# jibanCat/gp_dla_detection

Hardware: AMD Instinct MI355X
Metric: sample log-likelihoods/sec (n~1500,k=20) (higher is better)
Workload: dtype f64; 1 GPU; BASELINE configs[1]: synthetic spectra, fused Voigt + low-rank log-evidence sweep, HBM-resident; spectra_per_gpu=1000, pixels=1500, k=20, dla_samples=10000, num_lines=3, parallelism=spectra sharded over 1 GPU(s), RCCL all-gather of the 15-column posterior table

## Files before the change

gp_dla_detection_amd/_lib.py:

```python
from __future__ import annotations

import ctypes as C
import os
import subprocess

_HERE = os.path.dirname(os.path.abspath(__file__))
CSRC = os.path.join(_HERE, "csrc")
DEFAULT_LIB_PATH = os.path.join(CSRC, "libgpdla.so")


def lib_path() -> str:
    return os.environ.get("GPDLA_LIB_PATH") or DEFAULT_LIB_PATH

HIPCC_FLAGS = ["--offload-arch=gfx950", "-O3", "-ffp-contract=off", "-fPIC", "-shared",
               "-std=c++17", "-no-hip-rt", "-Wno-inline-asm"]

LEGACY_LIB_PATH = os.path.join(CSRC, "libgpdla_legacy.so")

_dp = C.POINTER(C.c_double)
_i64p = C.POINTER(C.c_int64)
_i32p = C.POINTER(C.c_int32)
_u8p = C.POINTER(C.c_uint8)
_u32p = C.POINTER(C.c_uint32)

# ... 146 lines not shown
    ("gpdla_batch_samples_device_ptr", C.c_int, [C.c_void_p, C.POINTER(C.c_void_p), _i64p, _i64p]),
    ("gpdla_context_last_sweep_ms", C.c_double, [C.c_void_p]),
    ("gpdla_context_set_timing", C.c_int, [C.c_void_p, C.c_int]),
    ("gpdla_process_batch_multi", C.c_int, [C.POINTER(Model), C.POINTER(Samples), C.POINTER(Spectra),
                                            _u32p, C.POINTER(Config), C.POINTER(ResultsMulti), C.c_int]),
    ("gpdla_batch_process_multi", C.c_int, [C.c_void_p, C.c_void_p, _u32p]),
    ("gpdla_batch_download_multi", C.c_int, [C.c_void_p, C.c_void_p, C.POINTER(ResultsMulti)]),
    ("gpdla_batch_summary_multi_device_ptr", C.c_int, [C.c_void_p, C.POINTER(C.c_void_p), _i64p, _i32p]),
    ("gpdla_batch_samples_multi_device_ptr", C.c_int, [C.c_void_p, C.POINTER(C.c_void_p),
                                                       C.POINTER(C.c_void_p), C.POINTER(C.c_void_p)]),
    ("gpdla_training_create", C.c_int, [C.c_int, C.c_int64, C.c_int64, _dp, _dp, _dp,
                                        C.POINTER(C.c_void_p)]),
    ("gpdla_training_objective", C.c_int, [C.c_void_p, _dp, C.c_int, _dp, _dp]),
    ("gpdla_training_set_lyseries", C.c_int, [C.c_void_p, C.c_int, _dp, _dp]),
    ("gpdla_training_destroy", None, [C.c_void_p]),
    ("gpdla_training_create_from_spectra", C.c_int, [C.c_int, C.POINTER(Spectra), C.POINTER(LearnConfig),
                                                     C.POINTER(C.c_void_p)]),
    ("gpdla_training_column_stats", C.c_int, [C.c_void_p, _dp, _dp, _i64p]),
    ("gpdla_training_pca_covariance", C.c_int, [C.c_void_p, C.c_int, _dp, _dp, _i64p]),
    ("gpdla_training_download", C.c_int, [C.c_void_p, _dp, _dp, _dp]),
    ("gpdla_stats_bin_posteriors", C.c_int, [C.c_int64, C.c_int64, _dp, C.c_int64, _dp, _dp, _dp, _dp, _dp, _dp, _dp,
                                             C.c_int, C.POINTER(BinRequest), C.POINTER(BinOutput), C.c_int]),
    ("gpdla_stats_poisson_binomial_cf", C.c_int, [C.c_int64, _i64p, _dp, _dp, _dp, C.c_int]),
    ("gpdla_model_spectra_validate", C.c_int, [C.POINTER(ModelSpectraRequest), C.c_int64, C.c_int64, C.c_int]),
    ("gpdla_batch_unmasked_counts", C.c_int, [C.c_void_p, C.c_void_p, _i64p]),
    ("gpdla_batch_model_spectra", C.c_int, [C.c_void_p, C.c_void_p, C.POINTER(ModelSpectraRequest),
                                            C.POINTER(ModelSpectra)]),
    ("gpdla_debug_profiles_ms", C.c_int, [C.c_void_p, C.c_void_p, _dp]),
    ("gpdla_model_mean", C.c_int, [C.POINTER(Model), C.c_int64, _dp, _i64p, _dp, _dp, C.c_int, C.c_int, C.c_int,
                                   C.c_double, C.c_double, _dp, C.c_int]),
    ("gpdla_mock_validate", C.c_int, [C.POINTER(MockRequest), C.c_int64]),
    ("gpdla_batch_draw_mocks", C.c_int, [C.c_void_p, C.c_void_p, C.POINTER(MockRequest), C.POINTER(MockSpectra)]),
    ("gpdla_debug_near_poly", C.c_int, [C.c_int, C.c_double, _dp, _dp]),
    ("gpdla_debug_prepared_rows", C.c_int, [C.c_void_p, C.c_void_p, C.c_int, C.c_int64, _dp, C.c_int64, _i64p]),
    ("gpdla_debug_philox4x32_10", None, [_u32p, _u32p, _u32p]),
    ("gpdla_debug_throw", C.c_int, [C.c_int]),
]

_lib = None


def host_sources() -> list:
    import re
    unit = os.path.join(CSRC, "gpdla.hip")
    with open(unit) as f:
        names = re.findall(r'^#include "(host_\w+\.hpp)"', f.read(), flags=re.M)
    return [unit] + [os.path.join(CSRC, n) for n in names]


def _build(out: str, extra_flags, force: bool, verbose: bool) -> str:
    import glob
    srcs = (host_sources() + glob.glob(os.path.join(CSRC, "*.hip")) + glob.glob(os.path.join(CSRC, "*.hpp"))
            + glob.glob(os.path.join(_HERE, "..", "include", "*.h")))
    if not force and os.path.exists(out):
        if all(os.path.getmtime(out) >= os.path.getmtime(s) for s in srcs):
            return out
    cmd = ["hipcc", *HIPCC_FLAGS, *extra_flags, os.path.join(CSRC, "gpdla.hip"), "-o", out]
    res = subprocess.run(cmd, capture_output=True, text=True)
    if verbose or res.returncode:
        print(res.stdout, res.stderr)
    if res.returncode:
        raise RuntimeError(f"hipcc failed building {os.path.basename(out)}:\n" + res.stderr)
    return out


def build(force: bool = False, verbose: bool = False) -> str:
# ... 49 lines not shown
```

gp_dla_detection_amd/csrc/host_common.hpp:

```cpp
#pragma once

namespace {

thread_local std::string t_error = "";

int fail(int code, const char *fmt, ...) {
  char buf[512];
  va_list ap;
  va_start(ap, fmt);
  vsnprintf(buf, sizeof(buf), fmt, ap);
  va_end(ap);
  t_error = buf;
  return code;
}

#define GPDLA_NO_THROW                                                                                    \
  catch (const std::bad_alloc &) { return fail(GPDLA_ERR_HOST, "out of host memory"); }                   \
  catch (const std::exception &e) { return fail(GPDLA_ERR_HOST, "unexpected C++ exception: %s", e.what()); } \
  catch (...) { return fail(GPDLA_ERR_HOST, "unexpected C++ exception"); }

#define HIP_TRY(expr)                                                                      \
  do {                                                                                     \
    hipError_t e_ = (expr);                                                                \
    if (e_ != hipSuccess)                                                                  \
// ... 37 lines not shown
  HIP_TRY(hipMalloc(reinterpret_cast<void **>(&d_near), g_near_host.size() * sizeof(double)));
  HIP_TRY(hipMemcpy(d_near, g_near_host.data(), g_near_host.size() * sizeof(double), hipMemcpyHostToDevice));
  LineTable t;
  t.near_poly = d_near;
#define GP_WL(i, wl, f, G, lead, gam) wl,
#define GP_LEAD(i, wl, f, G, lead, gam) lead,
#define GP_GAM(i, wl, f, G, lead, gam) gam,
#define GP_OSC(i, wl, f, G, lead, gam) f,
  const double wl[] = {GPDLA_LYMAN_SERIES(GP_WL)};
  const double lead[] = {GPDLA_LYMAN_SERIES(GP_LEAD)};
  const double gam[] = {GPDLA_LYMAN_SERIES(GP_GAM)};
  const double osc[] = {GPDLA_LYMAN_SERIES(GP_OSC)};
  const double taps[] = GPDLA_INSTRUMENT_PROFILE;
  const double sigma = GPDLA_GAUSS_SIGMA_CGS;
  for (int i = 0; i < kMaxLines; ++i) {
    t.wavelength_cm[i] = wl[i];
    t.leading[i] = lead[i];
    t.osc[i] = osc[i];
    t.y[i] = gam[i] / std::sqrt(2.0) / sigma;
    t.y2[i] = t.y[i] * t.y[i];
    t.cwing[i] = lead[i] * t.y[i];
    t.t2[i] = kE2 - 2.0 * t.y2[i];
    t.wing[i] = {GPDLA_SPEED_OF_LIGHT_CGS / wl[i] / 1e8 / (std::sqrt(2.0) * sigma), t.y2[i], t.cwing[i], 0.0};
  }
  for (int i = 0; i < 7; ++i) t.taps[i] = taps[i];
  t.c = GPDLA_SPEED_OF_LIGHT_CGS;
  t.inv_sqrt2_sigma = 1.0 / (std::sqrt(2.0) * sigma);
  t.inv_sqrt2pi_sigma = 1.0 / (std::sqrt(2.0 * 3.14159265358979323846) * sigma);
  HIP_TRY(hipMemcpyToSymbol(HIP_SYMBOL(g_lines), &t, sizeof(t)));
  if (device_id < 64) g_table_loaded[device_id] = true;
  return GPDLA_OK;
}

template <typename T>
int dev_alloc(T **p, size_t count) {
  *p = nullptr;
  if (count == 0) count = 1;
  HIP_TRY(hipMalloc(reinterpret_cast<void **>(p), count * sizeof(T)));
  return GPDLA_OK;
}

template <typename T>
int upload(T **p, const T *host, size_t count, hipStream_t st) {
  int rc = dev_alloc(p, count);
  if (rc) return rc;
  if (count) HIP_TRY(hipMemcpyAsync(*p, host, count * sizeof(T), hipMemcpyHostToDevice, st));
  return GPDLA_OK;
}

void dev_free(void *p) {
  if (p) (void)hipFree(p);
}

struct StreamDrain {
  hipStream_t stream;
  ~StreamDrain() { (void)hipStreamSynchronize(stream); }
};

template <typename T>
int reserve(T **p, size_t *cap, size_t count) {
  if (count == 0) count = 1;
  if (*p && *cap >= count) return GPDLA_OK;
  dev_free(*p);
  *p = nullptr;
  *cap = 0;
  int rc = dev_alloc(p, count);
// ... 60 lines not shown
```

gp_dla_detection_amd/csrc/host_sweep.hpp:

```cpp
#pragma once

namespace {

template <typename Args>
int launch_sweep_kernel(gpdla_context *c, void (*kernel)(Args), int threads, size_t lds, int samples_per_block,
                        int64_t num_quasars, Args args) {
  HIP_TRY(hipFuncSetAttribute(reinterpret_cast<const void *>(kernel), hipFuncAttributeMaxDynamicSharedMemorySize, (int)lds));
  args.blocks_per_quasar = (int32_t)((args.S + 1 + samples_per_block - 1) / samples_per_block);
  const int64_t nblocks = 8 * ((num_quasars + 7) / 8) * (int64_t)args.blocks_per_quasar;
  if (nblocks > 2147483647LL) return fail(GPDLA_ERR_UNSUPPORTED, "batch too large for one launch");
  hipLaunchKernelGGL(kernel, dim3((unsigned)nblocks), dim3(threads), lds, c->stream, args);
  HIP_TRY(hipGetLastError());
  return GPDLA_OK;
}

template <class F>
int dispatch_nd(int mode, F &&f) {
  switch (mode == 0 ? 1 : mode) {
    case 1: return f(std::integral_constant<int, 1>{});
    case 2: return f(std::integral_constant<int, 2>{});
    case 3: return f(std::integral_constant<int, 3>{});
    case 4: return f(std::integral_constant<int, 4>{});
    default: return fail(GPDLA_ERR_UNSUPPORTED, "max_dlas = %d > 4", mode);
  }
// ... 313 lines not shown
  if (k > 256) return fail(GPDLA_ERR_UNSUPPORTED, "k = %d too large", k);
  int rc = select_device(device_id);
  if (rc) return rc;
  double *buf = nullptr;
  const size_t nn = (size_t)n, ws = (size_t)k * (k + 1) / 2 + k + 2;
  const size_t n_in = 3 * nn + nn * k, total = n_in + ws + 2;
  if ((rc = dev_alloc(&buf, total))) return rc;
  std::vector<double> host(n_in);
  std::memcpy(host.data(), y, nn * sizeof(double));
  std::memcpy(host.data() + nn, mu, nn * sizeof(double));
  std::memcpy(host.data() + 2 * nn, d, nn * sizeof(double));
  std::memcpy(host.data() + 3 * nn, M, nn * k * sizeof(double));
  double *dy = buf, *dmu = dy + nn, *dd = dmu + nn, *dM = dd + nn, *dws = dM + nn * k, *dlp = dws + ws;
  int *d_status = reinterpret_cast<int *>(dlp + 1);
  hipError_t e = hipMemcpy(buf, host.data(), n_in * sizeof(double), hipMemcpyHostToDevice);
  double back[2] = {NAN, 0.0};
  if (e == hipSuccess) {
    hipLaunchKernelGGL(k_lowrank_single, dim3(1), dim3(256), 0, 0, dy, dmu, dM, dd, n, k, dws, dlp, d_status);
    e = hipGetLastError();
  }
  if (e == hipSuccess) e = hipMemcpy(back, dlp, 2 * sizeof(double), hipMemcpyDeviceToHost);
  dev_free(buf);
  if (e != hipSuccess) return fail(GPDLA_ERR_HIP, "gpdla_log_mvnpdf_low_rank: %s", hipGetErrorString(e));
  int status;
  std::memcpy(&status, &back[1], sizeof(int));
  *log_p = back[0];
  if (status) {
    *log_p = NAN;
    return fail(GPDLA_ERR_NOT_POSITIVE_DEFINITE, "B = I + M' D^-1 M is not positive definite");
  }
  return GPDLA_OK;
} GPDLA_NO_THROW

}

extern "C" int gpdla_debug_prepared_rows(gpdla_context *c, gpdla_batch *b, int multi, int64_t quasar,
                                         double *rows_out, int64_t capacity_rows, int64_t *num_rows_out) {
  if (!c || !b || b->ctx != c || !rows_out || !num_rows_out)
    return fail(GPDLA_ERR_INVALID_ARGUMENT, "null/mismatched argument");
  if (quasar < 0 || quasar >= b->nq) return fail(GPDLA_ERR_INVALID_ARGUMENT, "quasar %lld outside the batch", (long long)quasar);
  HIP_TRY(hipSetDevice(c->device_id));
  int rc = plan_records(c, b, b->k <= 20 ? kSlimRec : record_doubles(b->ntiles, 0), true);
  if (rc) return rc;
  if ((rc = launch_prepare(c, b, multi != 0))) return rc;
  QuasarMeta m;
  HIP_TRY(hipMemcpyAsync(&m, b->d_meta + quasar, sizeof(m), hipMemcpyDeviceToHost, c->stream));
  HIP_TRY(hipStreamSynchronize(c->stream));
  const int64_t n = std::min<int64_t>(m.n_u, capacity_rows);
  static_assert(sizeof(PixelRow) == 4 * sizeof(double), "rows_out is [n][4] doubles");
  if (n > 0) {
    HIP_TRY(hipMemcpyAsync(rows_out, b->d_pix + m.pix_off, (size_t)n * sizeof(PixelRow), hipMemcpyDeviceToHost, c->stream));
    HIP_TRY(hipStreamSynchronize(c->stream));
  }
  *num_rows_out = n;
  return GPDLA_OK;
}

#ifdef GPDLA_STAMP
extern "C" int gpdla_debug_stamps(unsigned long long *out) {
  unsigned long long zero[8] = {0, 0, 0, 0, 0, 0, 0, 0};
  if (hipDeviceSynchronize() != hipSuccess) return -1;
  if (hipMemcpyFromSymbol(out, HIP_SYMBOL(gpdla::g_stamps), sizeof(zero)) != hipSuccess) return -1;
  if (hipMemcpyToSymbol(HIP_SYMBOL(gpdla::g_stamps), zero, sizeof(zero)) != hipSuccess) return -1;
  return 0;
}
#endif
// ... 1 lines not shown
```

gp_dla_detection_amd/csrc/sweep_kernels.hpp:

```cpp
#pragma once
#include <hip/hip_runtime.h>
#include <stdint.h>

#include <type_traits>
#include <utility>

#include "faddeeva.hpp"
#include "near_tables.hpp"

namespace gpdla {

typedef double d4 __attribute__((ext_vector_type(4)));

typedef float f4 __attribute__((ext_vector_type(4)));

template <typename T> struct Mat;
template <> struct Mat<double> {
  using acc_t = d4;
  static __device__ __forceinline__ acc_t mfma(double a, double b, acc_t c) {
    return __builtin_amdgcn_mfma_f64_16x16x4f64(a, b, c, 0, 0, 0);
  }
  static __device__ __forceinline__ int sample_of(int jj, int r) { return jj + 4 * r; }
  static __device__ __forceinline__ int jj_of(int sample) { return sample & 3; }
  static __device__ __forceinline__ int reg_of(int sample) { return sample >> 2; }
};
template <> struct Mat<float> {
  using acc_t = f4;
  static __device__ __forceinline__ acc_t mfma(float a, float b, acc_t c) {
    return __builtin_amdgcn_mfma_f32_16x16x4f32(a, b, c, 0, 0, 0);
  }
  static __device__ __forceinline__ int sample_of(int jj, int r) { return 4 * jj + r; }
  static __device__ __forceinline__ int jj_of(int sample) { return sample >> 2; }
  static __device__ __forceinline__ int reg_of(int sample) { return sample & 3; }
};

constexpr int kMaxLines = 31;
constexpr int kSamplesPerWave = 16;
constexpr double kLog2Pi = 1.83787706640934534;

struct LineTable {
  double wavelength_cm[kMaxLines];
// ... 376 lines not shown
  int32_t blocks_per_quasar;
  int32_t k, tiles_w, ntiles, num_lines;
  double *sample_ll;
  double *ll_no_dla;
};

__device__ __forceinline__ double fast_rcp(double a) {
  const double r = __builtin_amdgcn_rcp(a);
  const double e = fma(-a, r, 1.0);
  return fma(r, e, r);
}

__device__ __forceinline__ double exp_nonpos(double x) {
  x = fmax(x, -800.0);
  const double n = rint(x * 1.4426950408889634);
  double r = fma(-n, 0.6931471803691238, x);
  r = fma(-n, 1.9082149292705877e-10, r);
  double p = 2.08767569878681e-09;
  p = fma(p, r, 2.505210838544172e-08);
  p = fma(p, r, 2.755731922398589e-07);
  p = fma(p, r, 2.755731922398589e-06);
  p = fma(p, r, 2.48015873015873e-05);
  p = fma(p, r, 0.0001984126984126984);
  p = fma(p, r, 0.001388888888888889);
  p = fma(p, r, 0.008333333333333333);
  p = fma(p, r, 0.041666666666666664);
  p = fma(p, r, 0.16666666666666666);
  p = fma(p, r, 0.5);
  p = fma(p, r, 1.0);
  p = fma(p, r, 1.0);
  return ldexp(p, (int)n);
}

constexpr double kE1 = 0x1.8000000000236p+0, kE2 = 0x1.dffffffd2a557p+1, kE3 = 0x1.a4000aa13fb7fp+3,
                 kE4 = 0x1.d86dfb645a1cbp+5, kE5 = 0x1.4be1ccccccccdp+8;

__device__ __forceinline__ double wing_core(double x2, double y2) {
  const double rho = fast_rcp(x2 + y2);
  double t = fma(kE5, rho, kE4);
  t = fma(t, rho, kE3);
  t = fma(t, rho, kE2);
  t = fma(t, rho, kE1);
  t = fma(t, rho, 1.0);
  t = fma(-2.0 * y2 * rho, rho, t);
  return rho * t;
}

__device__ __forceinline__ void glds16(const double *gsrc, double *lds_wave_base) {
  const uint32_t lds = __builtin_amdgcn_readfirstlane(
      (uint32_t)(uintptr_t)(__attribute__((address_space(3))) void *)lds_wave_base);
  asm volatile("s_mov_b32 m0, %1\n\ts_nop 0\n\tglobal_load_lds_dwordx4 %0, off"
               :
               : "v"(gsrc), "s"(lds)
               : "memory", "m0");
}
__device__ __forceinline__ void glds_wait() {
  __builtin_amdgcn_s_waitcnt(0x0F70);
  asm volatile("" ::: "memory");
}

constexpr int kRecordPoolPad = 8;
__device__ __forceinline__ void glds_quad(const double *gsrc, uint32_t lds, int count) {
  if (count >= 4)
    asm volatile("s_mov_b32 m0, %1\n\ts_nop 0\n\tglobal_load_lds_dwordx4 %0, off\n\t"
                 "global_load_lds_dwordx4 %0, off offset:1024\n\tglobal_load_lds_dwordx4 %0, off offset:2048\n\t"
                 "global_load_lds_dwordx4 %0, off offset:3072"
                 :
                 : "v"(gsrc), "s"(lds)
// ... 465 lines not shown
__device__ __forceinline__ uint32_t hi_word(double v) { return (uint32_t)__double2hiint(v); }

__device__ __forceinline__ double wing_sum3(double lamP, double msa, double msb, double msc, double cs,
                                            bool *near) {
  const double xa = fma(lamP, msa, -cs), xb = fma(lamP, msb, -cs), xc = fma(lamP, msc, -cs);
  const double sa = fma(xa, xa, g_lines.y2[0]), sb = fma(xb, xb, g_lines.y2[1]), sc = fma(xc, xc, g_lines.y2[2]);
  static_assert(__builtin_bit_cast(unsigned long long, 900.0) == 0x408C200000000000ull, "bits of 900.0");
  *near = min(min(hi_word(sa), hi_word(sb)), hi_word(sc)) < 0x408C2000u;
  const double pab = sa * sb, pbc = sb * sc, pac = sa * sc;
  const double rinv = fast_rcp(pab * sc);
  const double ra = rinv * pbc, rb = rinv * pac, rc = rinv * pab;
  double ta = ra * kE5 + kE4, tb = rb * kE5 + kE4, tc = rc * kE5 + kE4;
  ta = fma(ta, ra, kE3); tb = fma(tb, rb, kE3); tc = fma(tc, rc, kE3);
  ta = fma(ta, ra, g_lines.t2[0]); tb = fma(tb, rb, g_lines.t2[1]); tc = fma(tc, rc, g_lines.t2[2]);
  ta = fma(ta, ra, kE1); tb = fma(tb, rb, kE1); tc = fma(tc, rc, kE1);
  ta = fma(ta, ra, 1.0); tb = fma(tb, rb, 1.0); tc = fma(tc, rc, 1.0);
  return fma(g_lines.cwing[2], rc * tc, fma(g_lines.cwing[1], rb * tb, g_lines.cwing[0] * (ra * ta)));
}

__device__ __forceinline__ double wing_sum3_rcp4(double lamP, double msa, double msb, double msc, double cs,
                                                 bool *near, double d, double *inv_d) {
  const double xa = fma(lamP, msa, -cs), xb = fma(lamP, msb, -cs), xc = fma(lamP, msc, -cs);
  const double sa = fma(xa, xa, g_lines.y2[0]), sb = fma(xb, xb, g_lines.y2[1]), sc = fma(xc, xc, g_lines.y2[2]);
  *near = min(min(hi_word(sa), hi_word(sb)), hi_word(sc)) < 0x408C2000u;
  const double pab = sa * sb, pabc = pab * sc;
  const double rinv = fast_rcp(pabc * d);
  *inv_d = rinv * pabc;
  const double r3 = rinv * d;
  const double rc = r3 * pab, r2 = r3 * sc;
  const double ra = r2 * sb, rb = r2 * sa;
  double ta = ra * kE5 + kE4, tb = rb * kE5 + kE4, tc = rc * kE5 + kE4;
  ta = fma(ta, ra, kE3); tb = fma(tb, rb, kE3); tc = fma(tc, rc, kE3);
  ta = fma(ta, ra, g_lines.t2[0]); tb = fma(tb, rb, g_lines.t2[1]); tc = fma(tc, rc, g_lines.t2[2]);
  ta = fma(ta, ra, kE1); tb = fma(tb, rb, kE1); tc = fma(tc, rc, kE1);
  ta = fma(ta, ra, 1.0); tb = fma(tb, rb, 1.0); tc = fma(tc, rc, 1.0);
  return fma(g_lines.cwing[2], rc * tc, fma(g_lines.cwing[1], rb * tb, g_lines.cwing[0] * (ra * ta)));
}

constexpr int kRing2 = 33;
constexpr int kExpTab = 64;

struct ExpState {
  double r, tabv;
  int ni;
};
__device__ __forceinline__ ExpState exp_table_begin(double x, const double *tab) {
  ExpState e;
  const double nf = rint(x * 92.33248261689366);
  asm("v_cvt_i32_f64 %0, %1" : "=v"(e.ni) : "v"(nf));
  e.tabv = tab[e.ni & (kExpTab - 1)];
  e.r = fma(-nf, 0.010830424667801708, x);
  e.r = fma(-nf, 2.8447437476627285e-11, e.r);
  return e;
}
__device__ __forceinline__ double exp_table_end(const ExpState &e) {
  double p, c4 = 0.041666666666666664, c3 = 0.16666666666666666;
  asm("v_fma_f64 %0, %1, %2, %3" : "=v"(p) : "s"(0.008333333333333333), "v"(e.r), "v"(c4));
  asm("v_fma_f64 %0, %1, %2, %3" : "=v"(p) : "v"(p), "v"(e.r), "v"(c3));
  p = fma(p, e.r, 0.5);
  p = fma(p, e.r, 1.0);
  p = fma(p, e.r, 1.0);
  return ldexp(e.tabv * p, e.ni >> 6);
}
constexpr double kExpScale = 92.33248261689366;
__device__ __forceinline__ ExpState exp_table_begin_scaled(double t, const double *tab) {
  ExpState e;
// ... 591 lines not shown
```

gp_dla_detection_amd/csrc/sweep_slim_kernel.hpp:

```cpp
#pragma once
#include <type_traits>

#include "sweep_kernels.hpp"

namespace gpdla {

constexpr int kSlimExtras = 12;
constexpr int kSlimRec = 4 * kSlimExtras + 64;
constexpr int kSlimCH = 8;
constexpr int kSlimTilesW = 13;
constexpr int kSlimStepTiles = kSlimTilesW * 64;
constexpr int kSlimRingD = kSweepWaves * kSamplesPerWave * kRing2;
constexpr int kSlimTileBuf = kSlimCH * kSlimStepTiles;
constexpr int kSlimRawBuf = kSlimCH * kSlimRec;
constexpr int kSlimLand = 4 * 32 + 4 * 4;
constexpr int kSlimBlock = kSlimTileBuf + kSlimRawBuf;
constexpr int kSlimLdsDoubles = kSlimRingD + 2 * kSlimBlock + kSweepWaves * kSlimLand;
static_assert((kSlimBlock * 8) % 512 == 0, "both parities reachable with ds_read2st64 offsets");
static_assert(kSlimLdsDoubles * 8 == 160 * 1024, "the slim sweep uses the whole LDS of a CU");
static_assert((kSlimCH * kSlimRec) % 128 == 0, "a raw chunk is a whole number of KiB");

__host__ __device__ constexpr int slim_pair_i(int tile, int col) {
  if (tile < 8) {
    const int b = (col + tile) & 15;
    return col > b ? col : b;
  }
  if (tile == 8) {
    if (col < 8) return col + 8;
    const int l = col - 8;
    return l < 1 ? 16 : l < 3 ? 17 : l < 6 ? 18 : 19;
  }
  return 16 + (tile - 9);
}
__host__ __device__ constexpr int slim_pair_j(int tile, int col) {
  if (tile < 8) {
    const int b = (col + tile) & 15;
    return col > b ? b : col;
  }
  if (tile == 8) {
    if (col < 8) return col;
    const int l = col - 8;
    return 16 + (l < 1 ? 0 : l < 3 ? l - 1 : l < 6 ? l - 3 : l - 6);
  }
  return col;
}
__host__ __device__ constexpr int slim_pos(int tile, int col) {
  return slim_pair_i(tile, col) * (slim_pair_i(tile, col) + 1) / 2 + slim_pair_j(tile, col);
}

__global__ __launch_bounds__(256) void k_build_slim_records(BuildRecordsArgs a) {
  const int q = a.order[blockIdx.x / a.blocks_per_quasar];
  const int bq = blockIdx.x % a.blocks_per_quasar;
  const QuasarMeta m = a.meta[q];
  const int k = a.k;
  const int n_pad = m.n_u + 6;
  double *out = a.records + m.rec_off * (int64_t)kSlimRec;
  const int64_t total = (int64_t)(m.steps + 1) * kSlimRec;
  for (int64_t e = (int64_t)bq * 256 + threadIdx.x; e < total; e += (int64_t)a.blocks_per_quasar * 256) {
    const int step = (int)(e / kSlimRec), r = (int)(e - (int64_t)step * kSlimRec);
    double v = 0.0;
    if (r < 4 * kSlimExtras) {
      const int jj = r / kSlimExtras, f = r - jj * kSlimExtras;
      const int64_t row = m.pix_off + 4 * (int64_t)step + jj;
      if (f < 4) {
        const PixelRow px = a.pix[row];
        v = f == 0 ? px.y : f == 1 ? px.mu : f == 2 ? px.omega2 : px.nu;
      } else if (f < 8) {
        if (kXUColumn + (f - 4) < k) v = a.Mi[row * k + kXUColumn + (f - 4)];
      } else if (f < 10) {
        if (k == 20) v = a.Mi[row * k + 19] * a.Mi[row * k + 18 + (f - 8)];
      } else if (f == 10) {
        int P = 4 * (step + 3) + jj;
        if (P > n_pad - 1) P = n_pad - 1;
        v = a.lam_pad[m.lam_off + P];
      }
    } else {
      const int l = r - 4 * kSlimExtras, jj = l >> 4, col = l & 15;
      if (col < k) v = a.Mi[(m.pix_off + 4 * (int64_t)step + jj) * k + col];
    }
    out[e] = v;
  }
}

__device__ __forceinline__ ExpState exp_ring_begin_scaled(double t, const double *ring_pad) {
  ExpState e;
  const double nf = rint(t);
  asm("v_cvt_i32_f64 %0, %1" : "=v"(e.ni) : "v"(nf));
  e.tabv = ring_pad[(e.ni & (kExpTab - 1)) * kRing2];
  e.r = t - nf;
  return e;
}

__device__ __forceinline__ double slim_factor_pass(const d4 (&acc)[14], const double (&xw)[kXW],
                                                   const double (&xu)[kXU], int p, double *Eg, int lane, int k,
                                                   double quad_sum, double logd_sum, int n_kept,
                                                   int *sigma_out, bool *writer) {
  using ES = EpilogueShape<13, 1>;
  constexpr int voff = (13 + 1) * 16;
  constexpr int ncols = ES::stride(16);
  const int s = lane & 15, jj = lane >> 4;
  const int half = s >> 3;
  const int sigma = Mat<double>::sample_of(jj, ES::RPP * p + half);
  const double q_s = __shfl(quad_sum, sigma + 16 * jj);
  const double ld_s = __shfl(logd_sum, sigma + 16 * jj);
  double *e = Eg + (size_t)(jj * ES::RPP) * ncols;
#pragma unroll
  for (int cc = 0; cc < 14; ++cc) {
// ... 22 lines not shown
__global__ __launch_bounds__(512) void k_sweep_slim(SweepArgs a) {
  static_assert(LINES == 3 || LINES == 0, "three lines at compile time, or a run-time count");
  extern __shared__ double smem[];
  constexpr int WAVES = kSweepWaves, CH = kSlimCH;
  const int64_t xj = blockIdx.x >> 3;
  const int64_t pos = 8 * (xj / a.blocks_per_quasar) + (blockIdx.x & 7);
  const int bq = (int)(xj % a.blocks_per_quasar);
  if (pos >= a.nq) return;
  const int64_t q = a.order[pos];
  const QuasarMeta m = a.meta[q];
  if (m.status != 0) return;
  const int tid = threadIdx.x, wave = tid >> 6, lane = tid & 63;
  const int s = lane & 15, jj = lane >> 4;

  double *ring = smem;
  double *blocks = ring + kSlimRingD;
  double *land = blocks + 2 * kSlimBlock + wave * kSlimLand;
  const double *exp_pad = ring + 32;

  const int64_t slot0 = (int64_t)bq * (WAVES * kSamplesPerWave) + wave * kSamplesPerWave;
  const int64_t slot = slot0 + s;
  const bool is_sample = slot < a.S;
  const bool is_null = !is_sample;
  const int32_t sample = a.perm[is_sample ? slot : a.S - 1];
  const double z_dla = m.min_z_dla + (m.max_z_dla - m.min_z_dla) * a.offset_samples[sample];
  const double nhi = a.nhi_samples[sample];
  [[maybe_unused]] double mult_r[3];
  [[maybe_unused]] const double opz = 1 + z_dla, inv_opz = 1.0 / opz;
  [[maybe_unused]] const int L = LINES > 0 ? LINES : a.num_lines;
  if constexpr (LINES == 3) {
#pragma unroll
    for (int j = 0; j < 3; ++j) mult_r[j] = g_lines.c / (g_lines.wavelength_cm[j] * (1 + z_dla)) / 1e8;
  }
  if (tid < kExpTab) ring[tid * kRing2 + 32] = exp2((double)tid * (1.0 / kExpTab));
  double *my_ring = ring + (size_t)(wave * kSamplesPerWave + s) * kRing2 + jj;
  const double *lam = a.lam_pad + m.lam_off;
  const int n_pad = m.n_u + 6;
  const double nscale64 = -nhi * g_lines.inv_sqrt2pi_sigma * kInvSqrtPi * kExpScale;
  const double *rec_base = a.records + m.rec_off * (int64_t)kSlimRec;
  const int nchunks = (m.steps + CH - 1) / CH;

  const int wave_s = __builtin_amdgcn_readfirstlane(wave);
  const uint32_t raw_lds = __builtin_amdgcn_readfirstlane(lds_address(blocks + kSlimTileBuf));
  auto issue_chunk = [&](int c) {
    glds_chunk<CH * kSlimRec / 128, WAVES>(rec_base + (size_t)c * CH * kSlimRec,
                                           raw_lds + (uint32_t)(c & 1) * (uint32_t)(kSlimBlock * 8), wave_s, lane);
  };
  const double *land_src = rec_base + (size_t)wave_s * kSlimRec;
  const int src_rows = 4 * kSlimExtras + 16 * jj + 2 * (s & 7);
  const int src_x = kSlimExtras * (lane >> 1) + 4 + 2 * (lane & 1);
  auto issue_private = [&](int c) {
    const double *rec = land_src + (size_t)c * CH * kSlimRec;
    glds16(rec + src_rows, land);
    if (lane < 8) glds16(rec + src_x, land + 4 * 32);
  };
  const double *row = land + 32 * jj + s;
  const double *bc = land + 4 * 32 + 4 * jj;
  const double *a8 = s < 8 ? row : bc + (slim_pair_i(8, s) - 16);
  const double *b8 = s < 8 ? row + 8 : bc + (slim_pair_j(8, s) - 16);
  struct Operands {
    double mc, o[2], p8;
  };
  auto expand_load = [&](int t0, int t1, Operands &x) {
    x.mc = row[0];
#pragma unroll
    for (int t = t0; t < t1; ++t) {
      if (t == 8) {
        x.o[t - t0] = a8[0];
        x.p8 = b8[0];
      } else {
        x.o[t - t0] = t == 0 ? x.mc : t < 8 ? row[t] : bc[t - 9];
      }
    }
  };
  auto expand_store = [&](double *dst, int t0, int t1, const Operands &x) {
#pragma unroll
    for (int t = t0; t < t1; ++t) dst[t * 64] = (t == 8 ? x.p8 : x.mc) * x.o[t - t0];
  };
  double *const xd0 = blocks + (size_t)wave_s * kSlimStepTiles + lane;
  const double *const tb0 = blocks + lane;
  const double *const mb0 = blocks + kSlimTileBuf + kSlimExtras * jj;
  const double *const ub0 = blocks + kSlimTileBuf + 4 * kSlimExtras + lane;
  auto pinned = [](const double *p) {
    uint32_t v = lds_address(p);
    asm volatile("" : "+v"(v));
    return (double *)(__attribute__((address_space(3))) double *)(uintptr_t)v;
  };

  issue_private(0);
  issue_chunk(0);

  const double c_light = g_lines.c, inv_s = g_lines.inv_sqrt2_sigma;
  [[maybe_unused]] double ms_r[3];
  if constexpr (LINES == 3) {
#pragma unroll
    for (int j = 0; j < 3; ++j) ms_r[j] = mult_r[j] * inv_s;
  }
  const double cs = c_light * inv_s;
  auto optical_sum = [&](double lamP) -> double {
    if constexpr (LINES == 3) {
      bool near;
      double total = wing_sum3(lamP, ms_r[0], ms_r[1], ms_r[2], cs, &near);
      if (__builtin_expect(__any(near), 0)) total = total_near<3>(lamP, mult_r[0], mult_r[1], mult_r[2], nullptr, 3);
      return total;
    } else {
      bool near;
      double total = wing_sum_runtime(lamP * inv_opz, cs, L, &near);
      if (__builtin_expect(__any(near), 0)) total = total_near_at(lamP, opz, L);
      return total;
    }
  };

  __syncthreads();
  for (int c3 = 0; c3 < 3; ++c3) {
    const double lam0 = lam[min(4 * c3 + jj, n_pad - 1)];
    const double tot = optical_sum(lam0);
    const ExpState es0 = exp_ring_begin_scaled(nscale64 * tot, exp_pad);
    const double v = exp_table_end_scaled(es0);
    my_ring[4 * c3] = v;
    my_ring[4 * c3 + 16] = v;
  }

  d4 acc[14];
#pragma unroll
  for (int c = 0; c < 14; ++c) acc[c] = d4{0, 0, 0, 0};
  double quad_sum = 0.0, dprod = 1.0;
  double xw[kXW] = {0.0, 0.0}, xu[kXU] = {0.0, 0.0, 0.0, 0.0};
  int dexp = 0;
  const double tap0 = g_lines.taps[0], tap1 = g_lines.taps[1], tap2 = g_lines.taps[2], tap3 = g_lines.taps[3];

  glds_wait();
  {
    const double mc = row[0];
    for (int t = 0; t < kSlimTilesW; ++t)
      xd0[t * 64] = (t == 8 ? b8[0] : mc) * (t == 8 ? a8[0] : t == 0 ? mc : t < 8 ? row[t] : bc[t - 9]);
  }
  __builtin_amdgcn_s_waitcnt(0xC07F);
  if (nchunks > 1) issue_private(1);
  glds_wait();
  __syncthreads();

  for (int c = 0; c < nchunks; ++c) {
    __builtin_amdgcn_s_waitcnt(0x0F70);
    if (c + 1 < nchunks) issue_chunk(c + 1);
    const int par = (c & 1) * kSlimBlock;
    const double *tbuf = pinned(tb0 + par);
    const double *mine0 = pinned(mb0 + par);
    const double *ubuf = pinned(ub0 + par);
    double *xdst = pinned(xd0 + (kSlimBlock - par));
    double lam_next = 0.0;
#pragma unroll
    for (int tt = 0; tt < CH; ++tt) {
      const int rn = c * CH + tt;
      constexpr int kXS = 7;
      constexpr int kT0[7] = {0, 2, 4, 6, 8, 10, 12}, kT1[7] = {2, 4, 6, 8, 10, 12, 13};
      if (tt == kXS && c + 2 < nchunks) issue_private(c + 2);
      if (rn < m.steps) {
        const double *tl = tbuf + (size_t)tt * kSlimStepTiles;
        const double *mine = mine0 + (size_t)tt * kSlimRec;
        const int slot_p = (4 * tt) & 15;
        const int slot_w = (slot_p + 12) & 15;
        if (tt > 0) __builtin_amdgcn_s_waitcnt(0xC07F);
        const double lamP = tt == 0 ? mine[10] : lam_next;
        const double *g = my_ring + slot_p;
        const double g0 = g[0], g1 = g[1], g2 = g[2], g3 = g[3], g4 = g[4], g5 = g[5], g6 = g[6];
        const double2 p01 = *reinterpret_cast<const double2 *>(mine);
        const double2 p23 = *reinterpret_cast<const double2 *>(mine + 2);
        const double py = p01.x, pmu = p01.y, pom = p23.x, pnu = p23.y;
        __builtin_amdgcn_sched_barrier(0);
        double absorb = fma(g6, tap0, g0 * tap0);
        {
          double ab2 = fma(g5, tap1, g1 * tap1);
          absorb = fma(g2, tap2, absorb);
          ab2 = fma(g4, tap2, ab2);
          absorb = fma(g3, tap3, absorb) + ab2;
        }
        if (is_null) absorb = 1.0;
        const double a2 = absorb * absorb;
        const double d = fma(pom, a2, pnu);
        double inv_d;
        double total;
        if constexpr (LINES == 3) {
          bool near;
          total = wing_sum3_rcp4(lamP, ms_r[0], ms_r[1], ms_r[2], cs, &near, d, &inv_d);
#ifndef SLIM_EXP_NONEAR
          if (__builtin_expect(__any(near), 0)) total = total_near<3>(lamP, mult_r[0], mult_r[1], mult_r[2], nullptr, 3);
#endif
        } else {
          total = optical_sum(lamP);
          inv_d = fast_rcp(d);
        }
        const ExpState es = exp_ring_begin_scaled(nscale64 * total, exp_pad);
        __builtin_amdgcn_sched_barrier(0);
        double bop[14];
#pragma unroll
        for (int cc = 0; cc < kSlimTilesW; ++cc) bop[cc] = tl[cc * 64];
        bop[13] = ubuf[(size_t)tt * kSlimRec];
        __builtin_amdgcn_sched_barrier(0);
        const double raw = exp_table_end_scaled(es);
        my_ring[slot_w] = raw;
        my_ring[slot_w + 16] = raw;
        const double r = fma(-absorb, pmu, py);
        const double w = a2 * inv_d;
        const double ri = r * inv_d;
        const double u = absorb * ri;
        quad_sum = fma(r, ri, quad_sum);
        dprod *= d;
        if (tt & 1) {
          dexp += __builtin_amdgcn_frexp_exp(dprod);
          dprod = __builtin_amdgcn_frexp_mant(dprod);
        }
        Operands x;
        if (tt < kXS) expand_load(kT0[tt < kXS ? tt : 0], kT1[tt < kXS ? tt : 0], x);
        if (tt + 1 < CH) lam_next = mine[kSlimRec + 10];
        __builtin_amdgcn_sched_barrier(0);
#pragma unroll
        for (int cc = 0; cc < 14; ++cc)
          acc[cc] = __builtin_amdgcn_mfma_f64_16x16x4f64(cc < kSlimTilesW ? w : u, bop[cc], acc[cc], 0, 0, 0);
        {
          const double2 xp = *reinterpret_cast<const double2 *>(mine + 8);
          const double2 u01 = *reinterpret_cast<const double2 *>(mine + 4);
          const double2 u23 = *reinterpret_cast<const double2 *>(mine + 6);
          xw[0] = fma(w, xp.x, xw[0]);
          xw[1] = fma(w, xp.y, xw[1]);
          xu[0] = fma(u, u01.x, xu[0]);
          xu[1] = fma(u, u01.y, xu[1]);
          xu[2] = fma(u, u23.x, xu[2]);
          xu[3] = fma(u, u23.y, xu[3]);
        }
        if (tt < kXS) expand_store(xdst, kT0[tt < kXS ? tt : 0], kT1[tt < kXS ? tt : 0], x);
      }
    }
    glds_wait();
    __syncthreads();
  }

  double logd_sum = log(dprod) + (double)dexp * 0.6931471805599453;
  quad_sum += __shfl_xor(quad_sum, 16);
  quad_sum += __shfl_xor(quad_sum, 32);
  logd_sum += __shfl_xor(logd_sum, 16);
  logd_sum += __shfl_xor(logd_sum, 32);
#pragma unroll
  for (int x = 0; x < kXW; ++x) {
    xw[x] += __shfl_xor(xw[x], 16);
    xw[x] += __shfl_xor(xw[x], 32);
  }
#pragma unroll
  for (int x = 0; x < kXU; ++x) {
    xu[x] += __shfl_xor(xu[x], 16);
    xu[x] += __shfl_xor(xu[x], 32);
  }

  using ES = EpilogueShape<13, 1>;
  double *Eg = smem + (size_t)wave * ES::SPP * ES::stride(16);
#pragma unroll
  for (int p = 0; p < ES::PASSES; ++p) {
    int sigma;
    bool writer;
    const double ll = slim_factor_pass(acc, xw, xu, p, Eg, lane, a.k, quad_sum, logd_sum, m.n_kept, &sigma, &writer);
    const int64_t slot_s = slot0 + sigma;
    const int32_t sample_s = __shfl(sample, sigma + 16 * jj);
    if (writer) {
      if (slot_s < a.S) a.sample_ll[(int64_t)q * a.S + sample_s] = ll + m.ll_bias;
      else if (slot_s == a.S) a.ll_no_dla[q] = ll + m.ll_bias;
    }
  }
}

}
// ... 1 lines not shown
```

include/gpdla.h:

```cpp
#ifndef GPDLA_H
#define GPDLA_H

#include <stdint.h>

#ifdef __cplusplus
extern "C" {
#endif

typedef enum {
  GPDLA_OK = 0,
  GPDLA_ERR_INVALID_ARGUMENT = -1,
  GPDLA_ERR_NO_DEVICE = -2,
  GPDLA_ERR_HIP = -3,
  GPDLA_ERR_NOT_POSITIVE_DEFINITE = -4,
  GPDLA_ERR_UNSUPPORTED = -5,
  GPDLA_ERR_HOST = -6
} gpdla_status;

#define GPDLA_MAX_K 40
#define GPDLA_ABI_VERSION 6

int gpdla_abi_version(void);
const char *gpdla_last_error(void);

// ... 165 lines not shown
int gpdla_batch_samples_multi_device_ptr(gpdla_batch *batch, double **sample_ll_dla,
                                         double **sample_ll_lls, uint32_t **base_sample_inds);

typedef struct gpdla_training gpdla_training;
int gpdla_training_create(int device_id, int64_t num_quasars, int64_t num_pixels,
                          const double *centered_rest_fluxes, const double *lya_1pzs,
                          const double *rest_noise_variances, gpdla_training **out);
int gpdla_training_objective(gpdla_training *t, const double *x, int k, double *f, double *g);
int gpdla_training_set_lyseries(gpdla_training *t, int num_forest_lines, const double *all_transition_wavelengths,
                                const double *all_oscillator_strengths);
void gpdla_training_destroy(gpdla_training *t);

typedef struct {
  double min_lambda, dlambda;
  int64_t num_rest_pixels;
  double lya_wavelength;
  double max_noise_variance;
  double prev_tau_0, prev_beta;
  int32_t num_forest_lines;
} gpdla_learn_config;

int gpdla_training_create_from_spectra(int device_id, const gpdla_spectra *spectra, const gpdla_learn_config *config,
                                       gpdla_training **out);
int gpdla_training_column_stats(gpdla_training *t, double *mu, double *std, int64_t *count);
int gpdla_training_pca_covariance(gpdla_training *t, int complete_rows, double *cov, double *count,
                                  int64_t *rows_used);
int gpdla_training_download(gpdla_training *t, double *flux, double *lya, double *noise);

int gpdla_debug_near_poly(int line, double x, double *value_out, double *y_out);

int gpdla_debug_prepared_rows(gpdla_context *ctx, gpdla_batch *batch, int multi, int64_t quasar,
                              double *rows_out, int64_t capacity_rows, int64_t *num_rows_out);

void gpdla_debug_philox4x32_10(const uint32_t ctr[4], const uint32_t key[2], uint32_t out[4]);

int gpdla_debug_throw(int kind);

#define GPDLA_STATS_MAX_BINS 64
#define GPDLA_STATS_MAX_REQUESTS 4
#define GPDLA_STATS_KEPT_CAPACITY 8
typedef struct {
  int32_t quantity;
  int32_t num_bins;
  const double *edges;
  double z_lo, z_hi, lnhi_lo, lnhi_hi;
  int32_t histogram, moment, lowzcut;
  double p_thresh_sample, p_switch;
} gpdla_bin_request;
typedef struct {
  double *pois, *mean, *var;
  int32_t *kept_count;
  int32_t *kept_bin;
  double *kept_p;
} gpdla_bin_output;
int gpdla_stats_bin_posteriors(int64_t num_spectra, int64_t num_samples, const double *sample_log_likelihoods,
                               int64_t row_stride, const double *shift, const double *p_dla, const double *z_min,
                               const double *z_max, const double *upper_z, const double *offset_samples,
                               const double *log_nhi_samples, int num_requests, const gpdla_bin_request *requests,
                               gpdla_bin_output *outputs, int device_id);
int gpdla_stats_poisson_binomial_cf(int64_t num_segments, const int64_t *offsets, const double *p, double *logsum,
                                    double *argsum, int device_id);

#define GPDLA_SPECTRA_MAX_ABSORBERS 8
#define GPDLA_SPECTRA_MAP 1
#define GPDLA_SPECTRA_MOMENTS 2
#define GPDLA_SPECTRA_CONTINUUM 4
// ... 59 lines not shown
```

Baseline: 66.58 million evals/s.

## Add per-chunk wing tiers to skip near-line checks and idle waves in slim sweep

The slim sweep now classifies each chunk of 32 wavelengths per wave by its distance from the Lyman line centres, using lam min/max stashed in record padding and a wave-wide redshift range. Chunks that are provably far skip the near-line __any vote and total_near fallback. With GPDLA_SLIM_TRUNCATE defined they also use shorter Horner polynomials. Waves whose samples all lie past S skip the sweep arithmetic and only fill the exchange buffers. The cost is extra per-chunk min/max work in the record prep, tier ballots, a readfirstlane on cs, and a debug entry point for checking the tiers.

New measurement: 65.75 million evals/s. 0.988x the previous value.

```diff
diff --git a/gp_dla_detection_amd/_lib.py b/gp_dla_detection_amd/_lib.py
--- a/gp_dla_detection_amd/_lib.py
+++ b/gp_dla_detection_amd/_lib.py
@@ -202,6 +202,8 @@
     ("gpdla_mock_validate", C.c_int, [C.POINTER(MockRequest), C.c_int64]),
     ("gpdla_batch_draw_mocks", C.c_int, [C.c_void_p, C.c_void_p, C.POINTER(MockRequest), C.POINTER(MockSpectra)]),
     ("gpdla_debug_near_poly", C.c_int, [C.c_int, C.c_double, _dp, _dp]),
+    ("gpdla_debug_sweep_tiers", C.c_int, [_dp, C.c_int64, C.c_double, C.c_double, _dp, C.c_int64, _i32p, C.c_int64,
+                                          _i64p, _i64p]),
     ("gpdla_debug_prepared_rows", C.c_int, [C.c_void_p, C.c_void_p, C.c_int, C.c_int64, _dp, C.c_int64, _i64p]),
     ("gpdla_debug_philox4x32_10", None, [_u32p, _u32p, _u32p]),
     ("gpdla_debug_throw", C.c_int, [C.c_int]),
diff --git a/gp_dla_detection_amd/csrc/host_common.hpp b/gp_dla_detection_amd/csrc/host_common.hpp
--- a/gp_dla_detection_amd/csrc/host_common.hpp
+++ b/gp_dla_detection_amd/csrc/host_common.hpp
@@ -93,6 +93,16 @@
   return GPDLA_OK;
 }
 
+void host_wing_constants(double kms[3], double *cs) {
+#define GP_WL3(i, wl, f, G, lead, gam) wl,
+  const double wl[] = {GPDLA_LYMAN_SERIES(GP_WL3)};
+#undef GP_WL3
+  const double sigma = GPDLA_GAUSS_SIGMA_CGS;
+  for (int j = 0; j < 3; ++j) kms[j] = GPDLA_SPEED_OF_LIGHT_CGS / wl[j] / 1e8 / (std::sqrt(2.0) * sigma);
+  const double c = GPDLA_SPEED_OF_LIGHT_CGS, inv_sqrt2_sigma = 1.0 / (std::sqrt(2.0) * sigma);
+  *cs = c * inv_sqrt2_sigma;
+}
+
 template <typename T>
 int dev_alloc(T **p, size_t count) {
   *p = nullptr;
diff --git a/gp_dla_detection_amd/csrc/host_sweep.hpp b/gp_dla_detection_amd/csrc/host_sweep.hpp
--- a/gp_dla_detection_amd/csrc/host_sweep.hpp
+++ b/gp_dla_detection_amd/csrc/host_sweep.hpp
@@ -369,6 +369,49 @@
   return GPDLA_OK;
 } GPDLA_NO_THROW
 
+int gpdla_debug_sweep_tiers(const double *lam_padded, int64_t n_padded, double min_z_dla, double max_z_dla,
+                            const double *offset_samples, int64_t num_samples, int32_t *tiers_out, int64_t capacity,
+                            int64_t *num_waves_out, int64_t *num_chunks_out) try {
+  if (!lam_padded || !offset_samples || !tiers_out || !num_waves_out || !num_chunks_out || n_padded < 7 || num_samples < 1)
+    return fail(GPDLA_ERR_INVALID_ARGUMENT, "gpdla_debug_sweep_tiers: null argument, n_padded < 7 or no samples");
+  const int64_t S = num_samples, n_pad = n_padded, steps = (n_pad - 6 + 3) / 4, nchunks = (steps + kSlimCH - 1) / kSlimCH;
+  const int64_t waves = (S + 1 + kSamplesPerWave - 1) / kSamplesPerWave;
+  *num_waves_out = waves;
+  *num_chunks_out = nchunks;
+  if (capacity < waves * nchunks)
+    return fail(GPDLA_ERR_INVALID_ARGUMENT, "gpdla_debug_sweep_tiers: capacity %lld < %lld waves x %lld chunks",
+                (long long)capacity, (long long)waves, (long long)nchunks);
+  std::vector<int64_t> perm((size_t)S);
+  std::iota(perm.begin(), perm.end(), 0);
+  std::stable_sort(perm.begin(), perm.end(), [&](int64_t a, int64_t b) { return offset_samples[a] < offset_samples[b]; });
+  double kms[3], cs;
+  host_wing_constants(kms, &cs);
+  std::vector<uint32_t> lo_hi((size_t)nchunks), hi_hi((size_t)nchunks);
+  for (int64_t c = 0; c < nchunks; ++c) {
+    double lo = INFINITY, hi = -INFINITY;
+    for (int i = 0; i < kTierChunkPixels; ++i) {
+      const double l = lam_padded[std::min<int64_t>(kTierChunkPixels * c + kTierLookAhead + i, n_pad - 1)];
+      lo = fmin(lo, l);
+      hi = fmax(hi, l);
+    }
+    lo_hi[(size_t)c] = tier_hi_word(lo);
+    hi_hi[(size_t)c] = tier_hi_word(hi);
+  }
+  for (int64_t w = 0; w < waves; ++w) {
+    double zlo = INFINITY, zhi = -INFINITY;
+    for (int s = 0; s < kSamplesPerWave; ++s) {
+      const int64_t slot = w * kSamplesPerWave + s;
+      const double z_dla = min_z_dla + (max_z_dla - min_z_dla) * offset_samples[perm[(size_t)(slot < S ? slot : S - 1)]];
+      zlo = fmin(zlo, 1 + z_dla);
+      zhi = fmax(zhi, 1 + z_dla);
+    }
+    const TierBounds<kSweepTiers> tb = tier_bounds<kSweepTiers>(zlo, zhi, kms[0], kms[1], kms[2], cs);
+    for (int64_t c = 0; c < nchunks; ++c)
+      tiers_out[w * nchunks + c] = c < 64 ? tier_of(tb, lo_hi[(size_t)c], hi_hi[(size_t)c]) : 0;
+  }
+  return GPDLA_OK;
+} GPDLA_NO_THROW
+
 }
 
 extern "C" int gpdla_debug_prepared_rows(gpdla_context *c, gpdla_batch *b, int multi, int64_t quasar,
diff --git a/gp_dla_detection_amd/csrc/sweep_kernels.hpp b/gp_dla_detection_amd/csrc/sweep_kernels.hpp
--- a/gp_dla_detection_amd/csrc/sweep_kernels.hpp
+++ b/gp_dla_detection_amd/csrc/sweep_kernels.hpp
@@ -7,6 +7,7 @@
 
 #include "faddeeva.hpp"
 #include "near_tables.hpp"
+#include "sweep_tiers.hpp"
 
 namespace gpdla {
 
@@ -449,8 +450,6 @@
   return ldexp(p, (int)n);
 }
 
-constexpr double kE1 = 0x1.8000000000236p+0, kE2 = 0x1.dffffffd2a557p+1, kE3 = 0x1.a4000aa13fb7fp+3,
-                 kE4 = 0x1.d86dfb645a1cbp+5, kE5 = 0x1.4be1ccccccccdp+8;
 
 __device__ __forceinline__ double wing_core(double x2, double y2) {
   const double rho = fast_rcp(x2 + y2);
@@ -982,6 +981,35 @@
   double ta = ra * kE5 + kE4, tb = rb * kE5 + kE4, tc = rc * kE5 + kE4;
   ta = fma(ta, ra, kE3); tb = fma(tb, rb, kE3); tc = fma(tc, rc, kE3);
   ta = fma(ta, ra, g_lines.t2[0]); tb = fma(tb, rb, g_lines.t2[1]); tc = fma(tc, rc, g_lines.t2[2]);
+  ta = fma(ta, ra, kE1); tb = fma(tb, rb, kE1); tc = fma(tc, rc, kE1);
+  ta = fma(ta, ra, 1.0); tb = fma(tb, rb, 1.0); tc = fma(tc, rc, 1.0);
+  return fma(g_lines.cwing[2], rc * tc, fma(g_lines.cwing[1], rb * tb, g_lines.cwing[0] * (ra * ta)));
+}
+
+template <int LEVELS>
+__device__ __forceinline__ double wing_sum3_rcp4_far(double lamP, double msa, double msb, double msc, double cs,
+                                                     double d, double *inv_d) {
+  static_assert(LEVELS == 5 || LEVELS == 3 || LEVELS == 2, "Horner levels kept");
+  const double xa = fma(lamP, msa, -cs), xb = fma(lamP, msb, -cs), xc = fma(lamP, msc, -cs);
+  const double sa = fma(xa, xa, g_lines.y2[0]), sb = fma(xb, xb, g_lines.y2[1]), sc = fma(xc, xc, g_lines.y2[2]);
+  const double pab = sa * sb, pabc = pab * sc;
+  const double rinv = fast_rcp(pabc * d);
+  *inv_d = rinv * pabc;
+  const double r3 = rinv * d;
+  const double rc = r3 * pab, r2 = r3 * sc;
+  const double ra = r2 * sb, rb = r2 * sa;
+  double ta, tb, tc;
+  if constexpr (LEVELS == 5) {
+    ta = ra * kE5 + kE4; tb = rb * kE5 + kE4; tc = rc * kE5 + kE4;
+    ta = fma(ta, ra, kE3); tb = fma(tb, rb, kE3); tc = fma(tc, rc, kE3);
+  } else {
+    ta = tb = tc = kE3;
+  }
+  if constexpr (LEVELS >= 3) {
+    ta = fma(ta, ra, g_lines.t2[0]); tb = fma(tb, rb, g_lines.t2[1]); tc = fma(tc, rc, g_lines.t2[2]);
+  } else {
+    ta = g_lines.t2[0]; tb = g_lines.t2[1]; tc = g_lines.t2[2];
+  }
   ta = fma(ta, ra, kE1); tb = fma(tb, rb, kE1); tc = fma(tc, rc, kE1);
   ta = fma(ta, ra, 1.0); tb = fma(tb, rb, 1.0); tc = fma(tc, rc, 1.0);
   return fma(g_lines.cwing[2], rc * tc, fma(g_lines.cwing[1], rb * tb, g_lines.cwing[0] * (ra * ta)));
diff --git a/gp_dla_detection_amd/csrc/sweep_slim_kernel.hpp b/gp_dla_detection_amd/csrc/sweep_slim_kernel.hpp
--- a/gp_dla_detection_amd/csrc/sweep_slim_kernel.hpp
+++ b/gp_dla_detection_amd/csrc/sweep_slim_kernel.hpp
@@ -6,6 +6,7 @@
 namespace gpdla {
 
 constexpr int kSlimExtras = 12;
+constexpr int kSlimPad = 11;
 constexpr int kSlimRec = 4 * kSlimExtras + 64;
 constexpr int kSlimCH = 8;
 constexpr int kSlimTilesW = 13;
@@ -19,6 +20,12 @@
 static_assert((kSlimBlock * 8) % 512 == 0, "both parities reachable with ds_read2st64 offsets");
 static_assert(kSlimLdsDoubles * 8 == 160 * 1024, "the slim sweep uses the whole LDS of a CU");
 static_assert((kSlimCH * kSlimRec) % 128 == 0, "a raw chunk is a whole number of KiB");
+static_assert(kSlimCH * 4 == kTierChunkPixels, "a chunk evaluates the 32 wavelengths its range is taken over");
+#ifdef GPDLA_SLIM_TRUNCATE
+constexpr int kSlimTiers = kSweepTiers;
+#else
+constexpr int kSlimTiers = 1;
+#endif
 
 __host__ __device__ constexpr int slim_pair_i(int tile, int col) {
   if (tile < 8) {
@@ -73,6 +80,17 @@
         int P = 4 * (step + 3) + jj;
         if (P > n_pad - 1) P = n_pad - 1;
         v = a.lam_pad[m.lam_off + P];
+      } else if ((step & (kSlimCH - 1)) == 0) {
+        if (jj < 2) {
+          const int first = kTierChunkPixels * (step / kSlimCH) + kTierLookAhead;
+          double lo = INFINITY, hi = -INFINITY;
+          for (int i = 0; i < kTierChunkPixels; ++i) {
+            const double l = a.lam_pad[m.lam_off + min(first + i, n_pad - 1)];
+            lo = fmin(lo, l);
+            hi = fmax(hi, l);
+          }
+          v = jj ? hi : lo;
+        }
       }
     } else {
       const int l = r - 4 * kSlimExtras, jj = l >> 4, col = l & 15;
@@ -161,6 +179,27 @@
 #pragma unroll
     for (int j = 0; j < 3; ++j) mult_r[j] = g_lines.c / (g_lines.wavelength_cm[j] * (1 + z_dla)) / 1e8;
   }
+  [[maybe_unused]] uint64_t tier_mask[kSlimTiers];
+  if constexpr (LINES == 3) {
+    double zlo = opz, zhi = opz;
+#pragma unroll
+    for (int o = 1; o < kSamplesPerWave; o <<= 1) {
+      zlo = fmin(zlo, __shfl_xor(zlo, o));
+      zhi = fmax(zhi, __shfl_xor(zhi, o));
+    }
+    const TierBounds<kSlimTiers> tb = tier_bounds<kSlimTiers>(zlo, zhi, g_lines.wing[0].kms, g_lines.wing[1].kms,
+                                                              g_lines.wing[2].kms, g_lines.c * g_lines.inv_sqrt2_sigma);
+    int mine = 0;
+    if (lane < (m.steps + kSlimCH - 1) / kSlimCH) {
+      const double *r = a.records + (m.rec_off + (int64_t)lane * kSlimCH) * kSlimRec + kSlimPad;
+      mine = tier_of(tb, hi_word(r[0]), hi_word(r[kSlimExtras]));
+    }
+#ifdef GPDLA_SLIM_NO_FAR
+    mine = 0;
+#endif
+#pragma unroll
+    for (int t = 0; t < kSlimTiers; ++t) tier_mask[t] = __ballot(mine > t);
+  }
   if (tid < kExpTab) ring[tid * kRing2 + 32] = exp2((double)tid * (1.0 / kExpTab));
   double *my_ring = ring + (size_t)(wave * kSamplesPerWave + s) * kRing2 + jj;
   const double *lam = a.lam_pad + m.lam_off;
@@ -225,7 +264,8 @@
 #pragma unroll
     for (int j = 0; j < 3; ++j) ms_r[j] = mult_r[j] * inv_s;
   }
-  const double cs = c_light * inv_s;
+  const double cs = __hiloint2double(__builtin_amdgcn_readfirstlane(__double2hiint(c_light * inv_s)),
+                                     __builtin_amdgcn_readfirstlane(__double2loint(c_light * inv_s)));
   auto optical_sum = [&](double lamP) -> double {
     if constexpr (LINES == 3) {
       bool near;
@@ -269,22 +309,42 @@
   glds_wait();
   __syncthreads();
 
+#ifdef GPDLA_SLIM_NO_IDLE_SKIP
+  const bool idle_wave = false;
+#else
+  const bool idle_wave = (int64_t)bq * (WAVES * kSamplesPerWave) + wave_s * kSamplesPerWave > a.S;
+#endif
+  const int steps_w = idle_wave ? 0 : m.steps;
   for (int c = 0; c < nchunks; ++c) {
     __builtin_amdgcn_s_waitcnt(0x0F70);
     if (c + 1 < nchunks) issue_chunk(c + 1);
+    if (idle_wave && c + 1 < nchunks) {
+      double *dst = xd0 + (kSlimBlock - (c & 1) * kSlimBlock);
+      const double mc = row[0];
+      for (int t = 0; t < kSlimTilesW; ++t)
+        dst[t * 64] = (t == 8 ? b8[0] : mc) * (t == 8 ? a8[0] : t == 0 ? mc : t < 8 ? row[t] : bc[t - 9]);
+      __builtin_amdgcn_s_waitcnt(0xC07F);
+    }
     const int par = (c & 1) * kSlimBlock;
     const double *tbuf = pinned(tb0 + par);
     const double *mine0 = pinned(mb0 + par);
     const double *ubuf = pinned(ub0 + par);
     double *xdst = pinned(xd0 + (kSlimBlock - par));
     double lam_next = 0.0;
+    [[maybe_unused]] int tier = 0;
+    if constexpr (LINES == 3) {
+#pragma unroll
+      for (int t = 0; t < kSlimTiers; ++t) tier += (int)((tier_mask[t] >> (c & 63)) & 1);
+      if (c >= 64) tier = 0;
+      tier = __builtin_amdgcn_readfirstlane(tier);
+    }
 #pragma unroll
     for (int tt = 0; tt < CH; ++tt) {
       const int rn = c * CH + tt;
       constexpr int kXS = 7;
       constexpr int kT0[7] = {0, 2, 4, 6, 8, 10, 12}, kT1[7] = {2, 4, 6, 8, 10, 12, 13};
       if (tt == kXS && c + 2 < nchunks) issue_private(c + 2);
-      if (rn < m.steps) {
+      if (rn < steps_w) {
         const double *tl = tbuf + (size_t)tt * kSlimStepTiles;
         const double *mine = mine0 + (size_t)tt * kSlimRec;
         const int slot_p = (4 * tt) & 15;
@@ -310,11 +370,23 @@
         double inv_d;
         double total;
         if constexpr (LINES == 3) {
-          bool near;
-          total = wing_sum3_rcp4(lamP, ms_r[0], ms_r[1], ms_r[2], cs, &near, d, &inv_d);
+          int tier_k = tier;
+          asm volatile("" : "+s"(tier_k));
+#ifdef GPDLA_SLIM_TRUNCATE
+          if (tier_k == 2) {
+            total = wing_sum3_rcp4_far<3>(lamP, ms_r[0], ms_r[1], ms_r[2], cs, d, &inv_d);
+          } else if (tier_k == 3) {
+            total = wing_sum3_rcp4_far<2>(lamP, ms_r[0], ms_r[1], ms_r[2], cs, d, &inv_d);
+          } else
+#endif
+          {
+            bool near;
+            total = wing_sum3_rcp4(lamP, ms_r[0], ms_r[1], ms_r[2], cs, &near, d, &inv_d);
 #ifndef SLIM_EXP_NONEAR
-          if (__builtin_expect(__any(near), 0)) total = total_near<3>(lamP, mult_r[0], mult_r[1], mult_r[2], nullptr, 3);
+            if (tier_k == 0 && __builtin_expect(__any(near), 0))
+              total = total_near<3>(lamP, mult_r[0], mult_r[1], mult_r[2], nullptr, 3);
 #endif
+          }
         } else {
           total = optical_sum(lamP);
           inv_d = fast_rcp(d);
@@ -364,6 +436,7 @@
     __syncthreads();
   }
 
+  if (idle_wave) return;
   double logd_sum = log(dprod) + (double)dexp * 0.6931471805599453;
   quad_sum += __shfl_xor(quad_sum, 16);
   quad_sum += __shfl_xor(quad_sum, 32);
diff --git a/gp_dla_detection_amd/csrc/sweep_tiers.hpp b/gp_dla_detection_amd/csrc/sweep_tiers.hpp
--- /dev/null
+++ b/gp_dla_detection_amd/csrc/sweep_tiers.hpp
@@ -0,0 +1,76 @@
+#pragma once
+#include <cstdint>
+#include <cstring>
+
+#if defined(__HIPCC__) || defined(__CUDACC__)
+#define GPDLA_HD __host__ __device__
+#else
+#define GPDLA_HD
+#endif
+
+namespace gpdla {
+
+constexpr double kE1 = 0x1.8000000000236p+0, kE2 = 0x1.dffffffd2a557p+1, kE3 = 0x1.a4000aa13fb7fp+3,
+                 kE4 = 0x1.d86dfb645a1cbp+5, kE5 = 0x1.4be1ccccccccdp+8;
+
+constexpr int kSweepTiers = 3;
+constexpr double kTierS[kSweepTiers] = {900.0, 4.0e4, 8.0e5};
+constexpr double kTierMargin = 1.0 + 0x1p-19;
+constexpr double kTierX[kSweepTiers] = {30.00003, 200.0002, 894.4281};
+constexpr double kTierDrop = 0x1p-55;
+
+constexpr double tier_pow(double x, int n) { return n == 0 ? 1.0 : x * tier_pow(x, n - 1); }
+static_assert(kTierX[0] * kTierX[0] >= kTierS[0] * kTierMargin && kTierX[1] * kTierX[1] >= kTierS[1] * kTierMargin &&
+                  kTierX[2] * kTierX[2] >= kTierS[2] * kTierMargin,
+              "the |x| thresholds cover the s thresholds and their margin");
+static_assert(kTierS[0] >= 900.0, "tier 1: the near vote (s < 900) cannot pass");
+static_assert(kE4 / tier_pow(kTierS[1], 4) + kE5 / tier_pow(kTierS[1], 5) < kTierDrop,
+              "tier 2: the two dropped levels stay below 2^-55 of the kept sum");
+static_assert(kE3 / tier_pow(kTierS[2], 3) + kE4 / tier_pow(kTierS[2], 4) + kE5 / tier_pow(kTierS[2], 5) < kTierDrop,
+              "tier 3: the three dropped levels stay below 2^-55 of the kept sum");
+
+GPDLA_HD inline uint32_t tier_hi_word(double v) {
+  uint64_t b;
+  memcpy(&b, &v, sizeof b);
+  return (uint32_t)(b >> 32);
+}
+
+template <int TIERS>
+struct TierBounds {
+  uint32_t lo[TIERS][3], hi[TIERS][3];
+};
+template <int TIERS>
+GPDLA_HD inline TierBounds<TIERS> tier_bounds(double opz_min, double opz_max, double kms0, double kms1, double kms2,
+                                              double cs) {
+  static_assert(TIERS >= 1 && TIERS <= kSweepTiers, "tiers");
+  TierBounds<TIERS> b;
+  const double kms[3] = {kms0, kms1, kms2};
+  for (int t = 0; t < TIERS; ++t)
+    for (int j = 0; j < 3; ++j) {
+      b.lo[t][j] = tier_hi_word((cs - kTierX[t]) * opz_min / kms[j]);
+      b.hi[t][j] = tier_hi_word((cs + kTierX[t]) * opz_max / kms[j]);
+    }
+  return b;
+}
+
+template <int TIERS>
+GPDLA_HD inline int tier_of(const TierBounds<TIERS> &b, uint32_t lam_min_hi, uint32_t lam_max_hi) {
+  int tier = 0;
+  for (int t = 0; t < TIERS; ++t) {
+    bool clear = true;
+    for (int j = 0; j < 3; ++j) clear = clear && (lam_max_hi < b.lo[t][j] || lam_min_hi > b.hi[t][j]);
+    if (!clear) break;
+    tier = t + 1;
+  }
+  return tier;
+}
+
+GPDLA_HD inline int sweep_tier(double opz_min, double opz_max, double lam_min, double lam_max, double kms0,
+                               double kms1, double kms2, double cs) {
+  return tier_of(tier_bounds<kSweepTiers>(opz_min, opz_max, kms0, kms1, kms2, cs), tier_hi_word(lam_min),
+                 tier_hi_word(lam_max));
+}
+
+constexpr int kTierChunkPixels = 32, kTierLookAhead = 12;
+
+}
diff --git a/include/gpdla.h b/include/gpdla.h
--- a/include/gpdla.h
+++ b/include/gpdla.h
@@ -221,6 +221,10 @@
 int gpdla_debug_prepared_rows(gpdla_context *ctx, gpdla_batch *batch, int multi, int64_t quasar,
                               double *rows_out, int64_t capacity_rows, int64_t *num_rows_out);
 
+int gpdla_debug_sweep_tiers(const double *lam_padded, int64_t n_padded, double min_z_dla, double max_z_dla,
+                            const double *offset_samples, int64_t num_samples, int32_t *tiers_out, int64_t capacity,
+                            int64_t *num_waves_out, int64_t *num_chunks_out);
+
 void gpdla_debug_philox4x32_10(const uint32_t ctr[4], const uint32_t key[2], uint32_t out[4]);
 
 int gpdla_debug_throw(int kind);
```
